# thedonutfactory/zig-tfhe

Hardware: AMD Instinct MI355X
Metric: gate-bootstraps/sec (NAND, 128-bit params) at 1/2/4/8 MI355X; % HBM roofline (higher is better)
Workload: dtype f64; 1 GPU; 1024 NAND gate bootstraps per GPU per step, SECURITY_128_BIT (n=700, N=1024, L=3, Bg=2^6, t=9); global_batch=1024, params=128, parallelism=dp1

## Files before the change

### zig-tfhe_amd/csrc/tfhe_kernels.hip

```cpp
#include <algorithm>
#include <string>
#include <type_traits>

#include "tfhe_device.hpp"

namespace tfhe {


constexpr int BO_GATES = 8;
constexpr int BO_LDS_BUF = 2048 * 4;
constexpr int BO_LDS_AT = 1024 * 2;
constexpr int BO_LDS_TOTAL = BR_LDS_BK + BR_LDS_TW + BR_LDS_TWIST + BO_GATES * (BO_LDS_BUF + BO_LDS_AT);
static_assert(BO_LDS_TOTAL <= 160 * 1024, "octo form LDS");
constexpr int BO_LDS_BUF_AT = BR_LDS_BK + BR_LDS_TW + BR_LDS_TWIST;
static_assert(BO_LDS_BUF_AT % 4096 == 0 && BO_LDS_BUF % 4096 == 0, "gather_rot needs 4 KB-aligned buffers");

DEV void issue_bk_pair_async512(const double2 *__restrict__ src, double2 *slot, int tid) {
    const uint32_t base = (uint32_t)(size_t)(lds_void_t *)slot + (uint32_t)(tid & ~63) * 16;
    const uint32_t voff = (uint32_t)tid * 16;
#pragma unroll
    for (int k = 0; k < 4; k++) {
        const uint32_t dst = __builtin_amdgcn_readfirstlane(base + 512 * 16 * k);
        const double2 *piece = src + 512 * k;
        uint32_t keep;
        asm volatile(
            "s_mov_b32 %0, m0\n\ts_mov_b32 m0, %2\n\ts_nop 0\n\tglobal_load_lds_dwordx4 %1, %3\n\ts_mov_b32 m0, %0"
            : "=&s"(keep)
            : "v"(voff), "s"(dst), "s"(piece)
            : "memory");
    }
}

template <bool FU>
DEV void load_digits_row_regs(C2 *d, const uint32_t *tA, const uint32_t *tB, int row, int L, int bgbit,
                              const C2 *twist_t) {
    const bool from_a = row < L;
    const int level = from_a ? row : row - L;
#pragma unroll
    for (int q = 0; q < 8; q++) {
        const int m = br3(q);
        const uint32_t x0 = from_a ? tA[m] : tB[m], x1 = from_a ? tA[m + 8] : tB[m + 8];
        d[q] = twist_in<FU>(digit_f64_flipped(x0, level, bgbit), digit_f64_flipped(x1, level, bgbit), twist_t[64 * m]);
    }
}

template <bool FU>
DEV void mac_row_lds(C2 *fa, C2 *fb, const C2 *d, const double2 *bk, int t) {
    double2 k[2][2];
    k[0][0] = bk[t];
    k[0][1] = bk[64 + t];
#pragma unroll
    for (int q = 0; q < 8; q++) {
        const int c = q & 1;
        if (q + 1 < 8) {
            k[c ^ 1][0] = bk[(2 * q + 2) * 64 + t];
            k[c ^ 1][1] = bk[(2 * q + 3) * 64 + t];
        }
        const C2 x = d[q];
        const double2 ka = k[c][0], kb = k[c][1];
        if (FU) {
            fa[q] = c2(fmad(x.x, ka.x, fmad(-x.y, ka.y, fa[q].x)), fmad(x.x, ka.y, fmad(x.y, ka.x, fa[q].y)));
            fb[q] = c2(fmad(x.x, kb.x, fmad(-x.y, kb.y, fb[q].x)), fmad(x.x, kb.y, fmad(x.y, kb.x, fb[q].y)));
        } else {
            const C2 ta = c2(x.x * ka.x - x.y * ka.y, x.x * ka.y + x.y * ka.x);
            const C2 tb = c2(x.x * kb.x - x.y * kb.y, x.x * kb.y + x.y * kb.x);
            fa[q] = c2(fa[q].x + ta.x, fa[q].y + ta.y);
            fb[q] = c2(fb[q].x + tb.x, fb[q].y + tb.y);
        }
    }
}

template <int L, bool FU>
DEV void octo_rows(const uint32_t *tA, const uint32_t *tB, int bgbit, const LdsTwAtPass &T, const C2 *twist_t,
                   C2 *xb, int t, int tid, C2 *fa, C2 *fb, double2 *s_bk, uint32_t k0,
                   const double2 *__restrict__ bkd, uint32_t pairs) {
#pragma unroll 1
    for (int r = 0; r < 2 * L; r++) {
        const uint32_t k = k0 + (uint32_t)(r >> 1);
        C2 d[1][8];
        load_digits_row_regs<FU>(d[0], tA, tB, r, L, bgbit, twist_t);
        fft512<1, false, FU, LdsTwAtPass, true>(d, xb, T, t);
        if ((r & 1) == 0) {
            asm volatile("s_waitcnt vmcnt(0)" ::: "memory");
            __syncthreads();
            if (k + 1 < pairs)
                issue_bk_pair_async512(bkd + (size_t)((k + 1) / L) * L * 2048 + (size_t)((k + 1) % L) * 2048,
                                       s_bk + ((k + 1) & 1) * 2048, tid);
        }
        mac_row_lds<FU>(fa, fb, d[0], s_bk + (k & 1) * 2048 + (r & 1) * 1024, t);
    }
}

template <int L, bool SMALL, bool FU, bool TV = false>
__global__ __launch_bounds__(512, 1) void k_blind_rotate_octo(
    KParams P, DevTables TT, const uint8_t *__restrict__ ops, const uint32_t *__restrict__ in_a,
    const uint32_t *__restrict__ in_b, const uint32_t *__restrict__ idx, const uint32_t *__restrict__ testvec,
    const double2 *__restrict__ bkd, uint32_t *__restrict__ out, int out_mode, size_t B) {
    __shared__ __attribute__((aligned(16))) unsigned char smem[BO_LDS_TOTAL];
    const int tid = threadIdx.x;
    const int t = tid & 63;
    const int w = __builtin_amdgcn_readfirstlane(tid >> 6);
    double2 *s_bk = reinterpret_cast<double2 *>(smem);
    C2 *s_tw = reinterpret_cast<C2 *>(smem + BR_LDS_BK);
    C2 *s_twist = reinterpret_cast<C2 *>(smem + BR_LDS_BK + BR_LDS_TW);
    unsigned char *gbase = smem + BR_LDS_BK + BR_LDS_TW + BR_LDS_TWIST;
    uint32_t *s_buf = reinterpret_cast<uint32_t *>(gbase + w * BO_LDS_BUF);
    C2 *s_x = reinterpret_cast<C2 *>(s_buf);
    uint16_t *s_at = reinterpret_cast<uint16_t *>(gbase + BO_GATES * BO_LDS_BUF + w * BO_LDS_AT);

    const int n = P.n;
    const size_t g_raw = (size_t)blockIdx.x * BO_GATES + w;
    const bool valid = g_raw < B;
    const size_t g = valid ? g_raw : B - 1;
    const size_t ia = idx ? idx[2 * g] : g, ib = idx ? idx[2 * g + 1] : g;
    const uint32_t *A = in_a + ia * (size_t)(n + 1);
    const uint32_t *Bv = in_b ? in_b + ib * (size_t)(n + 1) : A;
    const int op = ops ? (int)ops[g] : 255;
    const uint32_t pairs = (uint32_t)n * L;
    if constexpr (TV) testvec = item_testvec(P, testvec, g);

    if (lds_layout_bad(smem)) {
        if (tid == 0) __hip_atomic_fetch_or(P.err, (uint32_t)DEV_ERR_LDS_LAYOUT, __ATOMIC_RELAXED, __HIP_MEMORY_SCOPE_AGENT);
        return;
    }
    issue_bk_pair_async512(bkd, s_bk, tid);
    for (int x = tid; x < 511; x += 512) s_tw[x] = TT.tw[x];
    for (int x = tid; x < 512; x += 512) s_twist[x] = TT.twist[x];
    int bt = 0;
    for (int i = t; i <= n; i += 64) {
        const uint32_t c = gate_combine(op, A[i], Bv[i], i == n);
        const uint32_t tl = (uint32_t)(((uint64_t)c + (1ull << 20)) >> 21);
        if (i < n) s_at[i] = (uint16_t)tl;
        else bt = 2048 - (int)tl;
    }
    bt = __builtin_amdgcn_readlane(bt, n & 63);
    uint32_t accA[16], accB[16];
#pragma unroll
    for (int m = 0; m < 16; m++) {
        accA[m] = rot_read(testvec, t + 64 * m, bt);
        accB[m] = rot_read(testvec + 1024, t + 64 * m, bt);
        s_buf[t + 64 * m] = accA[m];
        s_buf[1024 + t + 64 * m] = accB[m];
    }
    __syncthreads();
    LdsTwAtPass T;
    T.init(s_tw, TT);
    const C2 *twist_t = s_twist + t;
    int at_next = s_at[0];
    uint32_t near = NEAR_NONE;
    const uint32_t msbs = digit_msbs(L, P.bgbit);
    const uint32_t buf_base = (uint32_t)(size_t)(lds_void_t *)s_buf;

    for (int i = 0; i < n; i++) {
        const int at = __builtin_amdgcn_readfirstlane(at_next);
        at_next = s_at[i + 1 < n ? i + 1 : i];
        uint32_t tA[16], tB[16];
        uint32_t xb[16];
        gather_rot(buf_base, t, at, xb, tA, tB);
        __builtin_amdgcn_sched_barrier(0);
#pragma unroll
        for (int m = 0; m < 16; m++) {
            const uint32_t sg = gather_sign(xb[m]), off_s = P.offset - sg;
            tA[m] = tmp_word(tA[m], sg, off_s, accA[m], msbs);
            tB[m] = tmp_word(tB[m], sg, off_s, accB[m], msbs);
        }
        wave_sync();
        C2 fa[8], fb[8];
#pragma unroll
        for (int q = 0; q < 8; q++) {
            fa[q] = c2(0.0, 0.0);
            fb[q] = c2(0.0, 0.0);
        }
        octo_rows<L, FU>(tA, tB, P.bgbit, T, twist_t, s_x, t, tid, fa, fb, s_bk, (uint32_t)(L * i), bkd, pairs);
        inverse_and_add<SMALL, 64, true, FU>(fa, fb, s_x, T, twist_t, t, accA, accB, near);
        wave_sync();
#pragma unroll
        for (int m = 0; m < 16; m++) {
            s_buf[t + 64 * m] = accA[m];
            s_buf[1024 + t + 64 * m] = accB[m];
        }
        wave_sync();
    }
    if (FU) near_tie_flag(P, near, g, valid);

    if (!valid) return;
    if (out_mode == BR_OUT_LV1) {
        uint32_t *o = out + g * (size_t)1025;
        for (int j = t; j <= 1024; j += 64) o[j] = j == 0 ? s_buf[0] : j < 1024 ? 0u - s_buf[1024 - j] : s_buf[1024];
    } else if (out_mode == BR_OUT_LV0_EXTRACT2) {
        uint32_t *o = out + g * (size_t)(n + 1);
        for (int j = t; j <= n; j += 64) o[j] = j == 0 ? s_buf[0] : j < n ? 0u - s_buf[n - j] : s_buf[1024];
    } else {
        uint32_t *o = out + g * (size_t)2048;
        for (int j = t; j < 2048; j += 64) o[j] = s_buf[j];
    }
}



constexpr size_t BR_WIDE_MAX_ITEMS = 512;
constexpr int WIDE_INV_W0 = 2;
constexpr int WIDE_ROW45_PRIO = 1;

template <int L, bool SMALL, bool FU = false, int RC = 0, bool TV = false>
__global__ __launch_bounds__(512, 1) void k_blind_rotate_wide(
    KParams P, DevTables TT, const uint8_t *__restrict__ ops, const uint32_t *__restrict__ in_a,
    const uint32_t *__restrict__ in_b, const uint32_t *__restrict__ idx, const uint32_t *__restrict__ testvec,
    const double2 *__restrict__ bkd, uint32_t *__restrict__ out, int out_mode, size_t B) {
    __shared__ __attribute__((aligned(16))) C2 s_tw[512];
    __shared__ __attribute__((aligned(16))) C2 s_twist[512];
    __shared__ __attribute__((aligned(16))) C2 s_prod[2][2 * L][512];
    __shared__ __attribute__((aligned(16))) uint32_t s_acc[2048];
    __shared__ uint16_t s_at[1024];
    __shared__ int s_bt;
    __shared__ uint32_t s_rows[8];
    static_assert(!RC || L == 3, "row counters: L = 3");
    const int tid = threadIdx.x;
    const int t = tid & 63;
    const int w = __builtin_amdgcn_readfirstlane(tid >> 6);
    const int n = P.n;
    const size_t g = blockIdx.x;
    const size_t ia = idx ? idx[2 * g] : g, ib = idx ? idx[2 * g + 1] : g;
    const uint32_t *A = in_a + ia * (size_t)(n + 1);
    const uint32_t *Bv = in_b ? in_b + ib * (size_t)(n + 1) : A;
    const int op = ops ? (int)ops[g] : 255;
    if constexpr (TV) testvec = item_testvec(P, testvec, g);
    const size_t trgsw = (size_t)2 * L * 1024;

    for (int x = tid; x < 511; x += 512) s_tw[x] = TT.tw[x];
    for (int x = tid; x < 512; x += 512) s_twist[x] = TT.twist[x];
    if (RC && tid < 8) s_rows[tid] = 0u;
    const int row = RC && w < 4 ? w ^ 2 : w;
    if (w == 0) {
        for (int i = t; i <= n; i += 64) {
            uint32_t c = gate_combine(op, A[i], Bv[i], i == n);
            uint32_t tl = (uint32_t)(((uint64_t)c + (1ull << 20)) >> 21);
            if (i < n) s_at[i] = (uint16_t)tl;
            else s_bt = 2048 - (int)tl;
        }
    }
    double2 kr[8][2];
    if (w < 2 * L) {
#pragma unroll
        for (int q = 0; q < 8; q++)
#pragma unroll
            for (int h = 0; h < 2; h++) kr[q][h] = bkd[((size_t)row * 8 + q) * 128 + h * 64 + t];
    }
    __syncthreads();
    const int bt = __builtin_amdgcn_readfirstlane(s_bt);
    if (w < 2) {
#pragma unroll
        for (int m = 0; m < 16; m++) s_acc[w * 1024 + t + 64 * m] = rot_read(testvec + w * 1024, t + 64 * m, bt);
    }
    LdsTw T;
    T.init(s_tw, TT);
    const C2 *twist_t = s_twist + t;
    __syncthreads();
    const int ipoly = w - WIDE_INV_W0;
    const bool is_inv = ipoly == 0 || ipoly == 1;
    const bool pf_late = !RC && w < 2 * L && !is_inv;
    uint32_t accr[16];
    if (is_inv) {
#pragma unroll
        for (int m = 0; m < 16; m++) accr[m] = s_acc[ipoly * 1024 + t + 64 * m];
    }

    if (RC ? (w == 0 || w == 1) : (w == 4 || w == 5)) __builtin_amdgcn_s_setprio(WIDE_ROW45_PRIO);
    uint32_t fail = 0;
    const uint32_t spin_cap = P.spin_cap ? P.spin_cap : BR_SPIN_CAP_DEFAULT;
    int at_next = s_at[0];
    uint32_t near = NEAR_NONE;
    PhaseProf pp;
    pp.start();
    for (int i = 0; i < n; i++) {
        pp.mark(0);
        const int at = __builtin_amdgcn_readfirstlane(at_next);
        at_next = s_at[i + 1 < n ? i + 1 : i];
        if (w < 2 * L) {
            const int poly = row >= L ? 1 : 0;
            const int level = row - poly * L;
            const uint32_t *pa = s_acc + poly * 1024;
            uint32_t rot[16], own[16];
            pp.mark(8);
            const int rb = (t - at) & 2047;
#pragma unroll
            for (int m = 0; m < 16; m++) {
                rot[m] = pa[(rb + 64 * m) & 1023];
                own[m] = pa[t + 64 * m];
            }
            __builtin_amdgcn_sched_barrier(0);
            pp.mark(9);
            C2 d[1][8];
            const uint32_t msbs = digit_msbs(L, P.bgbit);
#pragma unroll
            for (int q = 0; q < 8; q++) {
                const int m = br3(q);
                const bool n0 = ((rb + 64 * m) & 1024) != 0, n1 = ((rb + 64 * (m + 8)) & 1024) != 0;
                const uint32_t x0 = ((n0 ? 0u - rot[m] : rot[m]) - own[m] + P.offset) ^ msbs;
                const uint32_t x1 = ((n1 ? 0u - rot[m + 8] : rot[m + 8]) - own[m + 8] + P.offset) ^ msbs;
                d[0][q] = twist_in<FU>(digit_f64_flipped(x0, level, P.bgbit), digit_f64_flipped(x1, level, P.bgbit),
                                       twist_t[64 * m]);
            }
            pp.mark(10);
            fft512<1, false, FU>(d, s_prod[0][row], T, t);
            pp.mark(11);
#pragma unroll
            for (int q = 0; q < 8; q++) {
                s_prod[0][row][t + 64 * q] = cmul_bk<FU>(d[0][q], kr[q][0]);
                s_prod[1][row][t + 64 * q] = cmul_bk<FU>(d[0][q], kr[q][1]);
            }
            if (RC) {
                __builtin_amdgcn_sched_barrier(0);
                counter_add(s_rows + row);
            }
            pp.mark(14);
            if (i + 1 < n && !pf_late) wide_prefetch(kr, bkd + (size_t)(i + 1) * trgsw, row, t);
        }
        if (RC) {
            if (is_inv) {
                C2 fs[8];
                pp.mark(2);
#pragma unroll
                for (int r = 0; r < 2 * L; r++) {
                    uint32_t f = 0;
                    spin_until_ge<1>(s_rows + r, (uint32_t)i + 1u, spin_cap, f);
                    fail |= f;
                    __builtin_amdgcn_sched_barrier(0);
#pragma unroll
                    for (int q = 0; q < 8; q++) {
                        const C2 tq = s_prod[ipoly][r][t + 64 * q];
                        fs[q] = r == 0 ? tq : c2(fs[q].x + tq.x, fs[q].y + tq.y);
                    }
                }
                pp.mark(4);
                C2 e[1][8];
#pragma unroll
                for (int q = 0; q < 8; q++) e[0][q] = fs[br3(q)];
                C2 twr[8];
#pragma unroll
                for (int q = 0; q < 8; q++) twr[q] = twist_t[64 * q];
                pp.mark(12);
                fft512<1, true, FU>(e, s_prod[ipoly][0], T, t);
                pp.mark(13);
                uint32_t *pa = s_acc + ipoly * 1024;
#pragma unroll
                for (int q = 0; q < 8; q++) {
                    double re, im;
                    untwist_out<false, FU>(e[0][q], twr[q], re, im);
                    accr[q] += to_torus<SMALL, FU>(re, near);
                    accr[q + 8] += to_torus<SMALL, FU>(im, near);
                    pa[t + 64 * q] = accr[q];
                    pa[t + 64 * q + 512] = accr[q + 8];
                }
            }
            pp.mark(5);
            __syncthreads();
            continue;
        }
        pp.mark(1);
        __syncthreads();
        pp.mark(2);
        const int f = t + 64 * w;
        C2 fa = s_prod[0][0][f], fb = s_prod[1][0][f];
#pragma unroll
        for (int r = 1; r < 2 * L; r++) {
            const C2 ta = s_prod[0][r][f], tb = s_prod[1][r][f];
            fa = c2(fa.x + ta.x, fa.y + ta.y);
            fb = c2(fb.x + tb.x, fb.y + tb.y);
        }
        s_prod[0][0][f] = fa;
        s_prod[0][1][f] = fb;
        pp.mark(3);
        __syncthreads();
        pp.mark(4);
        if (pf_late && i + 1 < n) wide_prefetch(kr, bkd + (size_t)(i + 1) * trgsw, row, t);
        if (is_inv) {
            C2 e[1][8];
#pragma unroll
            for (int q = 0; q < 8; q++) e[0][q] = s_prod[0][ipoly][t + 64 * br3(q)];
            C2 twr[8];
#pragma unroll
            for (int q = 0; q < 8; q++) twr[q] = twist_t[64 * q];
            pp.mark(12);
            fft512<1, true, FU>(e, s_prod[0][ipoly], T, t);
            pp.mark(13);
            uint32_t *pa = s_acc + ipoly * 1024;
#pragma unroll
            for (int q = 0; q < 8; q++) {
                double re, im;
                untwist_out<false, FU>(e[0][q], twr[q], re, im);
                accr[q] += to_torus<SMALL, FU>(re, near);
                accr[q + 8] += to_torus<SMALL, FU>(im, near);
                pa[t + 64 * q] = accr[q];
                pa[t + 64 * q + 512] = accr[q + 8];
            }
        }
        pp.mark(5);
        __syncthreads();
    }
    pp.mark(6);
#ifdef TFHE_PHASE_PROF
    if (t == 0)
        pp.flush(g_phase_cycles + w * 16, 16);
#endif
    if (RC) report_wait_failure(P, fail, DEV_ERR_GATE_WAIT);
    if (FU) near_tie_flag(P, near, g, true);

    if (w != 0) return;
    if (out_mode == BR_OUT_LV1) {
        uint32_t *o = out + g * (size_t)1025;
        for (int j = t; j <= 1024; j += 64) o[j] = j == 0 ? s_acc[0] : j < 1024 ? 0u - s_acc[1024 - j] : s_acc[1024];
    } else if (out_mode == BR_OUT_LV0_EXTRACT2) {
        uint32_t *o = out + g * (size_t)(n + 1);
        for (int j = t; j <= n; j += 64) o[j] = j == 0 ? s_acc[0] : j < n ? 0u - s_acc[n - j] : s_acc[1024];
    } else {
        uint32_t *o = out + g * (size_t)2048;
        for (int j = t; j < 2048; j += 64) o[j] = s_acc[j];
    }
}


template <int T, int G>
__global__ __launch_bounds__(256) void k_key_switch_sel(KParams P, const uint32_t *__restrict__ lv1,
                                                        const uint32_t *__restrict__ ksk,
                                                        uint32_t *__restrict__ out, size_t B) {
    const size_t g0 = (size_t)blockIdx.y * G;
    const int w = blockIdx.x * 256 + threadIdx.x;
    const int lane = threadIdx.x & 63;
    const int n1 = P.n + 1;
    const bool active = w < n1;
    const int wc = active ? w : 0;
    uint32_t res[G];
#pragma unroll
    for (int g = 0; g < G; g++) res[g] = (w == P.n && g0 + g < B) ? lv1[(g0 + g) * 1025 + 1024] : 0u;
    const uint32_t prec = 1u << (32 - (1 + 2 * T));
    const size_t rs = (size_t)P.ks_stride;
    const size_t stride_i = (size_t)T * 4 * rs;
    const uint32_t *rows0 = ksk + wc;
    for (int i0 = 0; i0 < 1024; i0 += 64) {
        uint32_t pkv[G];
#pragma unroll
        for (int g = 0; g < G; g++) {
            const uint32_t a = (g0 + g < B) ? lv1[(g0 + g) * 1025 + i0 + lane] : 0u;
            pkv[g] = (a + prec) >> (32 - 2 * T);
        }
        for (int ii = 0; ii < 64; ii++) {
            const uint32_t *rows = rows0 + (size_t)(i0 + ii) * stride_i;
            uint32_t r[T][3];
#pragma unroll
            for (int j = 0; j < T; j++)
#pragma unroll
                for (int k = 0; k < 3; k++) r[j][k] = rows[(size_t)(4 * j + k + 1) * rs];
#pragma unroll
            for (int g = 0; g < G; g++) {
                const uint32_t pk = __builtin_amdgcn_readlane(pkv[g], ii);
#pragma unroll
                for (int j = 0; j < T; j++) {
                    const uint32_t k = (pk >> (2 * (T - 1 - j))) & 3u;
                    const uint32_t v = (k & 2u) ? ((k & 1u) ? r[j][2] : r[j][1]) : ((k & 1u) ? r[j][0] : 0u);
                    res[g] -= v;
                }
            }
        }
    }
    if (active) {
#pragma unroll
        for (int g = 0; g < G; g++)
            if (g0 + g < B) out[(g0 + g) * n1 + w] = res[g];
    }
}

template <int T, int G>
__global__ __launch_bounds__(256) void k_key_switch_gather(KParams P, const uint32_t *__restrict__ lv1,
                                                           const uint32_t *__restrict__ ksk,
                                                           uint32_t *__restrict__ out, size_t B) {
    const size_t g0 = (size_t)blockIdx.y * G;
    const int w = blockIdx.x * 256 + threadIdx.x;
    const int lane = threadIdx.x & 63;
    const int n1 = P.n + 1;
    const bool active = w < n1;
    const int wc = active ? w : 0;
    const int basebit = P.basebit, base = 1 << basebit;
    uint32_t res[G];
#pragma unroll
    for (int g = 0; g < G; g++) res[g] = (w == P.n && g0 + g < B) ? lv1[(g0 + g) * 1025 + 1024] : 0u;
    const uint32_t prec = 1u << (32 - (1 + basebit * T));
    const size_t rs = (size_t)P.ks_stride;
    const size_t stride_i = (size_t)T * base * rs;
    const uint32_t *rows0 = ksk + wc;
    for (int i0 = 0; i0 < 1024; i0 += 64) {
        uint32_t pkv[G];
#pragma unroll
        for (int g = 0; g < G; g++) {
            const uint32_t a = (g0 + g < B) ? lv1[(g0 + g) * 1025 + i0 + lane] : 0u;
            pkv[g] = (a + prec) >> (32 - basebit * T);
        }
#pragma unroll 2
        for (int ii = 0; ii < 64; ii++) {
            const uint32_t *rows = rows0 + (size_t)(i0 + ii) * stride_i;
            uint32_t v[G][T];
#pragma unroll
            for (int g = 0; g < G; g++) {
                const uint32_t pk = __builtin_amdgcn_readlane(pkv[g], ii);
#pragma unroll
                for (int j = 0; j < T; j++) {
                    const uint32_t k = (pk >> (basebit * (T - 1 - j))) & (uint32_t)(base - 1);
                    v[g][j] = rows[(size_t)(base * j + k) * rs];
                }
            }
#pragma unroll
            for (int g = 0; g < G; g++)
#pragma unroll
                for (int j = 0; j < T; j++) res[g] -= v[g][j];
        }
    }
    if (active) {
#pragma unroll
        for (int g = 0; g < G; g++)
            if (g0 + g < B) out[(g0 + g) * n1 + w] = res[g];
    }
}

constexpr int KG_WAVES = 8;
constexpr int KG_ITEMS = 64 * KG_WAVES;
typedef int kg_v4i __attribute__((ext_vector_type(4)));
typedef int kg_v16i __attribute__((ext_vector_type(16)));

__host__ __device__ __forceinline__ int kg_cb(int basebit) { return basebit == 2 ? 8 : 4; }
__host__ __device__ __forceinline__ int kg_ksteps(int basebit) { return basebit == 2 ? 1 : 4; }
__host__ __device__ __forceinline__ int kg_blocks(int n_in, int basebit) { return (n_in + kg_cb(basebit) - 1) / kg_cb(basebit); }
static size_t ks_gemm_bytes_w(int out_w, int n_in, int t, int basebit) {
    const size_t w32 = (size_t)(out_w + 31) / 32;
    return (size_t)t * kg_blocks(n_in, basebit) * w32 * kg_ksteps(basebit) * 4 * 1024;
}
size_t ks_gemm_bytes(const KParams &P, int n_in, int t, int basebit) { return ks_gemm_bytes_w(P.n + 1, n_in, t, basebit); }
__global__ void k_ksk_to_gemm(KParams P, const uint32_t *__restrict__ ksk, uint32_t *__restrict__ kg, size_t words,
                              int n_in, int t, int basebit, int out_w, int row_stride) {
    const size_t x = (size_t)blockIdx.x * blockDim.x + threadIdx.x;
    if (x >= words) return;
    const int w32 = (out_w + 31) / 32, nib = kg_blocks(n_in, basebit), ks = kg_ksteps(basebit);
    const int base = 1 << basebit;
    const int q = (int)(x & 3), lane = (int)((x >> 2) & 63), b = (int)((x >> 8) & 3);
    size_t r = x >> 10;
    const int st = (int)(r % ks);
    r /= ks;
    const int wt = (int)(r % w32);
    r /= w32;
    const int ib = (int)(r % nib), j = (int)(r / nib);
    const int h = lane >> 5, c = lane & 31, w = 32 * wt + c;
    const size_t rs = (size_t)row_stride;
    uint32_t v = 0;
#pragma unroll
    for (int e4 = 0; e4 < 4; e4++) {
        const int e = 4 * q + e4;
        const int i = basebit == 2 ? 8 * ib + 4 * h + (e >> 2) : 4 * ib + st;
        const int k = basebit == 2 ? (e & 3) : 16 * h + e;
        const uint32_t word =
            (w < out_w && i < n_in) ? ksk[((size_t)(base * t) * i + (size_t)base * j + k) * rs + w] : 0u;
        v |= (((word >> (8 * b)) & 255u) ^ 128u) << (8 * e4);
    }
    kg[x] = v;
}

template <int N>
DEV void kg_wait() {
    static_assert(N >= 0 && N <= 15, "kg_wait");
#define KG_W(n_) if constexpr (N == n_) asm volatile("s_waitcnt vmcnt(" #n_ ")" ::: "memory");
    KG_W(0) KG_W(1) KG_W(2) KG_W(3) KG_W(4) KG_W(5) KG_W(6) KG_W(7)
    KG_W(8) KG_W(9) KG_W(10) KG_W(11) KG_W(12) KG_W(13) KG_W(14) KG_W(15)
#undef KG_W
}

template <int T, int BASEBIT>
__global__ __launch_bounds__(64 * KG_WAVES, 1) void k_key_switch_gemm(KParams P, const uint32_t *__restrict__ lv1,
                                                                   const uint32_t *__restrict__ kg,
                                                                   uint32_t *__restrict__ part, size_t B,
                                                                   int ib_per_split, int n_in, int in_stride,
                                                                   int out_w) {
    constexpr int CB = BASEBIT == 2 ? 8 : 4;
    constexpr int KS = BASEBIT == 2 ? 1 : 4;
    constexpr int STEP_BYTES = KS * 4 * 1024;
    constexpr int WORDS_BYTES = CB * KG_ITEMS * 4;
    constexpr int WORD_DMAS = CB / 4;
    constexpr int BUF_BYTES = T * STEP_BYTES + WORDS_BYTES;
    constexpr int STAGES = 3 * BUF_BYTES <= 160 * 1024 ? 3 : 2;
    constexpr int LOADER_DMAS = T * KS + WORD_DMAS;
    constexpr int OTHER_DMAS = WORD_DMAS;
    static_assert(STAGES * BUF_BYTES <= 160 * 1024, "gemm key-switch LDS");
    __shared__ __attribute__((aligned(16))) unsigned char smem[STAGES * BUF_BYTES];
    const int tid = threadIdx.x, lane = tid & 63;
    const int v = __builtin_amdgcn_readfirstlane(tid >> 6);
    const bool loader = v < 4;
    const int w32 = (out_w + 31) / 32;
    const int wt = blockIdx.x;
    const int nib = kg_blocks(n_in, BASEBIT);
    const int ib_lo = blockIdx.z * ib_per_split, ib_hi = min(nib, ib_lo + ib_per_split);
    const size_t m_wg = (size_t)blockIdx.y * KG_ITEMS;
    const int h = lane >> 5, c = lane & 31;
    const uint32_t *a_src[WORD_DMAS];
#pragma unroll
    for (int r = 0; r < WORD_DMAS; r++) {
        const size_t m = m_wg + (CB == 8 ? 256 * r + (tid >> 1) : tid);
        a_src[r] = lv1 + (m < B ? m : B - 1) * (size_t)in_stride + (CB == 8 ? 4 * (tid & 1) : 0);
    }
    const uint32_t lds0 = (uint32_t)(size_t)(lds_void_t *)smem;
    auto issue = [&](int ib, int slot) {
        const uint32_t base = lds0 + slot * BUF_BYTES;
        if (loader) {
#pragma unroll
            for (int j = 0; j < T; j++)
#pragma unroll
                for (int st = 0; st < KS; st++) {
                    const uint32_t *src = kg + ((((size_t)j * nib + ib) * w32 + wt) * KS + st) * 1024 + tid * 4;
                    const uint32_t dst =
                        __builtin_amdgcn_readfirstlane(base + j * STEP_BYTES + st * 4096 + (tid & ~63) * 16);
                    uint32_t keep;
                    asm volatile(
                        "s_mov_b32 %0, m0\n\ts_mov_b32 m0, %2\n\ts_nop 0\n\tglobal_load_lds_dwordx4 %1, off\n\ts_mov_b32 m0, %0"
                        : "=&s"(keep)
                        : "v"(src), "s"(dst)
                        : "memory");
                }
        }
#pragma unroll
        for (int r = 0; r < WORD_DMAS; r++) {
            const uint32_t dst =
                __builtin_amdgcn_readfirstlane(base + T * STEP_BYTES + r * 256 * 32 + (tid & ~63) * 16);
            uint32_t keep;
            asm volatile(
                "s_mov_b32 %0, m0\n\ts_mov_b32 m0, %2\n\ts_nop 0\n\tglobal_load_lds_dwordx4 %1, off\n\ts_mov_b32 m0, %0"
                : "=&s"(keep)
                : "v"(a_src[r] + CB * ib), "s"(dst)
                : "memory");
        }
    };
    kg_v16i acc[2][4];
#pragma unroll
    for (int s = 0; s < 2; s++)
#pragma unroll
        for (int b = 0; b < 4; b++) acc[s][b] = kg_v16i{};
    const uint32_t prec = 1u << (32 - (1 + BASEBIT * T));
#pragma unroll
    for (int k = 0; k < STAGES - 1; k++)
        if (ib_lo + k < ib_hi) issue(ib_lo + k, k);
    for (int ib = ib_lo; ib < ib_hi; ib++) {
        const int slot = (ib - ib_lo) % STAGES;
        const int ahead = min(STAGES - 2, ib_hi - 1 - ib);
        if (ahead == 1) {
            if (loader) kg_wait<LOADER_DMAS>();
            else kg_wait<OTHER_DMAS>();
        } else {
            kg_wait<0>();
        }
        __syncthreads();
        if (ib + STAGES - 1 < ib_hi) issue(ib + STAGES - 1, (slot + STAGES - 1) % STAGES);
        const unsigned char *buf = smem + slot * BUF_BYTES;
        const uint32_t *words = reinterpret_cast<const uint32_t *>(buf + T * STEP_BYTES);
        if constexpr (BASEBIT == 2) {
            uint32_t pk[2][4];
#pragma unroll
            for (int s = 0; s < 2; s++) {
                const kg_v4i wv = *reinterpret_cast<const kg_v4i *>(words + (64 * v + 32 * s + c) * 8 + 4 * h);
#pragma unroll
                for (int q = 0; q < 4; q++) pk[s][q] = ((uint32_t)wv[q] + prec) >> (32 - 2 * T);
            }
#pragma unroll
            for (int j = 0; j < T; j++) {
                kg_v4i a[2];
#pragma unroll
                for (int s = 0; s < 2; s++)
#pragma unroll
                    for (int q = 0; q < 4; q++)
                        a[s][q] = (int)(1u << (8u * ((pk[s][q] >> (2 * (T - 1 - j))) & 3u)));
#pragma unroll
                for (int b = 0; b < 4; b++) {
                    const kg_v4i bf = *reinterpret_cast<const kg_v4i *>(buf + j * STEP_BYTES + b * 1024 + lane * 16);
#pragma unroll
                    for (int s = 0; s < 2; s++)
                        acc[s][b] = __builtin_amdgcn_mfma_i32_32x32x32_i8(a[s], bf, acc[s][b], 0, 0, 0);
                }
            }
        } else {
            uint32_t pk[2][4];
#pragma unroll
            for (int s = 0; s < 2; s++) {
                const kg_v4i wv = *reinterpret_cast<const kg_v4i *>(words + (64 * v + 32 * s + c) * 4);
#pragma unroll
                for (int q = 0; q < 4; q++) pk[s][q] = ((uint32_t)wv[q] + prec) >> (32 - BASEBIT * T);
            }
#pragma unroll
            for (int j = 0; j < T; j++)
#pragma unroll
                for (int st = 0; st < KS; st++) {
                    kg_v4i a[2];
#pragma unroll
                    for (int s = 0; s < 2; s++) {
                        const uint32_t d = (pk[s][st] >> (BASEBIT * (T - 1 - j))) & 31u;
                        const uint32_t one = 1u << (8u * (d & 3u));
                        const int word = (int)(d >> 2) - 4 * h;
#pragma unroll
                        for (int q = 0; q < 4; q++) a[s][q] = word == q ? (int)one : 0;
                    }
#pragma unroll
                    for (int b = 0; b < 4; b++) {
                        const kg_v4i bf = *reinterpret_cast<const kg_v4i *>(buf + j * STEP_BYTES + st * 4096 +
                                                                            b * 1024 + lane * 16);
#pragma unroll
                        for (int s = 0; s < 2; s++)
                            acc[s][b] = __builtin_amdgcn_mfma_i32_32x32x32_i8(a[s], bf, acc[s][b], 0, 0, 0);
                    }
                }
        }
    }
    const int n1 = out_w;
    uint32_t *pz = part + (size_t)blockIdx.z * B * n1;
    const int w = 32 * wt + c;
    const size_t m_base = m_wg + 64 * v;
#pragma unroll
    for (int s = 0; s < 2; s++)
#pragma unroll
        for (int reg = 0; reg < 16; reg++) {
            const size_t m = m_base + 32 * s + (reg & 3) + 8 * (reg >> 2) + 4 * h;
            const uint32_t val = (uint32_t)acc[s][0][reg] + ((uint32_t)acc[s][1][reg] << 8) +
                                 ((uint32_t)acc[s][2][reg] << 16) + ((uint32_t)acc[s][3][reg] << 24);
            if (m < B && w < n1) pz[m * n1 + w] = val;
        }
}

__global__ void k_ks_gemm_reduce(KParams P, const uint32_t *__restrict__ lv1, const uint32_t *__restrict__ part,
                                 uint32_t *__restrict__ out, size_t B, int splits, int n_in, int in_stride, int t,
                                 int basebit) {
    const int n1 = P.n + 1;
    const size_t x = (size_t)blockIdx.x * blockDim.x + threadIdx.x;
    if (x >= B * n1) return;
    const size_t m = x / n1;
    const int w = (int)(x % n1);
    uint32_t r = (uint32_t)(kg_cb(basebit) * kg_blocks(n_in, basebit) * t) * 128u * 0x01010101u;
    for (int z = 0; z < splits; z++) r += part[(size_t)z * B * n1 + x];
    out[x] = (w == P.n ? lv1[m * (size_t)in_stride + n_in] : 0u) - r;
}

__global__ void k_ksk_zero_k0(uint32_t *__restrict__ ksk, int rs, int base, size_t groups) {
    size_t idx = (size_t)blockIdx.x * blockDim.x + threadIdx.x;
    if (idx >= groups * rs) return;
    size_t grp = idx / rs, x = idx % rs;
    ksk[grp * base * rs + x] = 0u;
}

constexpr int KL_CHUNK = 32;
constexpr int KL_WAVES = 4;
constexpr int KL_CHUNK_WIDE = 44;
constexpr int KL_WAVES_WIDE = 8;

template <int T, int BASEBIT, int CHUNK = KL_CHUNK, int WAVES = KL_WAVES, int GW = 1>
__global__ __launch_bounds__(64 * WAVES) void k_key_switch_lanes(KParams P, const uint32_t *__restrict__ lv1,
                                                          const uint32_t *__restrict__ ksk,
                                                          uint32_t *__restrict__ out, size_t B, int n_in,
                                                          int in_stride) {
    constexpr int BASE = 1 << BASEBIT;
    constexpr int PIECES = CHUNK / 4;
    constexpr int SLOTS = T * PIECES * BASE;
    constexpr int NDMA = (SLOTS + 63) / 64;
    constexpr int BUF = NDMA * 64 + 16;
    constexpr int RING = 2 * BUF;
    constexpr int RED = WAVES * CHUNK * 64;
    constexpr int LDS_BYTES = (RING * 16 * WAVES > RED * 4) ? RING * 16 * WAVES : RED * 4;
    static_assert(LDS_BYTES <= 160 * 1024, "key-switch LDS");
    __shared__ __attribute__((aligned(16))) unsigned char smem[LDS_BYTES];
    const int lane = threadIdx.x & 63;
    const int w = __builtin_amdgcn_readfirstlane(threadIdx.x >> 6);
    constexpr int IW = WAVES / GW;
    static_assert(WAVES % GW == 0, "GW divides WAVES");
    const int gw = w % GW, iw = w / GW;
    uint4 *ring = reinterpret_cast<uint4 *>(smem) + w * RING;
    const size_t g_raw = (size_t)blockIdx.y * (64 * GW) + gw * 64 + lane;
    const bool valid = g_raw < B;
    const size_t g = valid ? g_raw : B - 1;
    const int w0 = blockIdx.x * CHUNK;
    const size_t rs = (size_t)P.ks_stride;
    const size_t step_i = (size_t)BASE * T * rs;
    const int per = (n_in + IW - 1) / IW;
    const int ilo = min(n_in, iw * per), ihi = min(n_in, ilo + per);
    uint32_t src_off[NDMA];
#pragma unroll
    for (int c = 0; c < NDMA; c++) {
        const int sl = min(c * 64 + lane, SLOTS - 1);
        const int k = sl % BASE, piece = (sl / BASE) % PIECES, j = sl / (BASE * PIECES);
        src_off[c] = (uint32_t)((BASE * j + k) * rs + w0 + 4 * piece);
    }
    const uint32_t ring_lds = (uint32_t)(size_t)(lds_void_t *)ring;
    const uint32_t *a_src = lv1 + g * (size_t)in_stride;
    auto issue = [&](int i, int which) {
        const uint32_t *r = ksk + (size_t)i * step_i;
#pragma unroll
        for (int c = 0; c < NDMA; c++) {
            const uint32_t dst = __builtin_amdgcn_readfirstlane(ring_lds + (which * BUF + c * 64) * 16);
            uint32_t keep;
            asm volatile(
                "s_mov_b32 %0, m0\n\ts_mov_b32 m0, %2\n\ts_nop 0\n\tglobal_load_lds_dwordx4 %1, off\n\ts_mov_b32 m0, %0"
                : "=&s"(keep)
                : "v"(r + src_off[c]), "s"(dst)
                : "memory");
        }
        const uint32_t dst = __builtin_amdgcn_readfirstlane(ring_lds + (which * BUF + NDMA * 64) * 16);
        uint32_t keep;
        asm volatile(
            "s_mov_b32 %0, m0\n\ts_mov_b32 m0, %2\n\ts_nop 0\n\tglobal_load_lds_dword %1, off\n\ts_mov_b32 m0, %0"
            : "=&s"(keep)
            : "v"(a_src + i), "s"(dst)
            : "memory");
    };
    const uint32_t prec = 1u << (32 - (1 + BASEBIT * T));
    uint32_t acc[CHUNK];
#pragma unroll
    for (int x = 0; x < CHUNK; x++) acc[x] = 0u;
    if (ilo < ihi) issue(ilo, 0);
    for (int i = ilo; i < ihi; i++) {
        const int cur = (i - ilo) & 1;
        asm volatile("s_waitcnt vmcnt(0)" ::: "memory");
        wave_sync();
        if (i + 1 < ihi) issue(i + 1, cur ^ 1);
        const uint4 *buf = ring + cur * BUF;
        const uint32_t a = reinterpret_cast<const uint32_t *>(buf + NDMA * 64)[lane];
        const uint32_t pk = (a + prec) >> (32 - BASEBIT * T);
#pragma unroll
        for (int j = 0; j < T; j++) {
            const uint32_t k = (pk >> (BASEBIT * (T - 1 - j))) & (uint32_t)(BASE - 1);
            const uint4 *sl = buf + j * PIECES * BASE + k;
#pragma unroll
            for (int pc = 0; pc < PIECES; pc++) {
                const uint4 v = sl[pc * BASE];
                acc[4 * pc + 0] -= v.x;
                acc[4 * pc + 1] -= v.y;
                acc[4 * pc + 2] -= v.z;
                acc[4 * pc + 3] -= v.w;
            }
        }
        asm volatile("s_waitcnt lgkmcnt(0)" ::: "memory");
    }
    __syncthreads();
    uint32_t *red = reinterpret_cast<uint32_t *>(smem);
#pragma unroll
    for (int x = 0; x < CHUNK; x++) red[(w * CHUNK + x) * 64 + lane] = acc[x];
    __syncthreads();
    const int n1 = P.n + 1;
    for (int x = iw; x < CHUNK; x += IW) {
        uint32_t r = 0u;
#pragma unroll
        for (int v = 0; v < IW; v++) r += red[((v * GW + gw) * CHUNK + x) * 64 + lane];
        const int word = w0 + x;
        if (valid && word < n1) out[g * n1 + word] = (word == P.n ? a_src[n_in] : 0u) + r;
    }
}

constexpr int KS_RING_DEPTH = 4;
template <int N>
DEV void wait_vmcnt_le() {
    static_assert(N >= 0 && N < 64, "vmcnt field");
    __builtin_amdgcn_s_waitcnt((N & 15) | (7 << 4) | (15 << 8) | ((N >> 4) << 14));
}
template <int T, int BASEBIT, int CHUNK, int GW, int DEPTH>
__global__ __launch_bounds__(64 * GW) void k_key_switch_ring(KParams P, const uint32_t *__restrict__ lv1,
                                                           const uint32_t *__restrict__ ksk,
                                                           uint32_t *__restrict__ out, size_t B, int n_in,
                                                           int in_stride) {
    constexpr int BASE = 1 << BASEBIT;
    constexpr int PIECES = CHUNK / 4;
    constexpr int SLOTS = T * PIECES * BASE;
    static_assert(SLOTS % 64 == 0, "whole DMA instructions");
    constexpr int NDMA = SLOTS / 64;
    constexpr int MINE = (NDMA + GW - 1) / GW;
    constexpr int BUF = SLOTS + GW * 16;
    static_assert(DEPTH >= 3 && (MINE + 1) * (DEPTH - 2) < 64, "ring depth");
    __shared__ __attribute__((aligned(16))) uint4 ring[DEPTH * BUF];
    const int lane = threadIdx.x & 63;
    const int gw = __builtin_amdgcn_readfirstlane(threadIdx.x >> 6);
    const size_t g_raw = (size_t)blockIdx.y * (64 * GW) + gw * 64 + lane;
    const bool valid = g_raw < B;
    const size_t g = valid ? g_raw : B - 1;
    const int w0 = blockIdx.x * CHUNK;
    const size_t rs = (size_t)P.ks_stride;
    const size_t step_i = (size_t)BASE * T * rs;
    uint32_t src_off[MINE];
#pragma unroll
    for (int cc = 0; cc < MINE; cc++) {
        const int sl = ((cc * GW + gw) % NDMA) * 64 + lane;
        const int k = sl % BASE, piece = (sl / BASE) % PIECES, j = sl / (BASE * PIECES);
        src_off[cc] = (uint32_t)((BASE * j + k) * rs + w0 + 4 * piece);
    }
    const uint32_t ring_lds = (uint32_t)(size_t)(lds_void_t *)ring;
    const uint32_t *a_src = lv1 + g * (size_t)in_stride;
    auto issue = [&](int i, int slot) {
        const uint32_t *r = ksk + (size_t)i * step_i;
#pragma unroll
        for (int cc = 0; cc < MINE; cc++) {
            const uint32_t dst = __builtin_amdgcn_readfirstlane(ring_lds + (slot * BUF + ((cc * GW + gw) % NDMA) * 64) * 16);
            uint32_t keep;
            asm volatile(
                "s_mov_b32 %0, m0\n\ts_mov_b32 m0, %2\n\ts_nop 0\n\tglobal_load_lds_dwordx4 %1, off\n\ts_mov_b32 m0, %0"
                : "=&s"(keep)
                : "v"(r + src_off[cc]), "s"(dst)
                : "memory");
        }
        const uint32_t dst = __builtin_amdgcn_readfirstlane(ring_lds + (slot * BUF + SLOTS + gw * 16) * 16);
        uint32_t keep;
        asm volatile(
            "s_mov_b32 %0, m0\n\ts_mov_b32 m0, %2\n\ts_nop 0\n\tglobal_load_lds_dword %1, off\n\ts_mov_b32 m0, %0"
            : "=&s"(keep)
            : "v"(a_src + i), "s"(dst)
            : "memory");
    };
    const uint32_t prec = 1u << (32 - (1 + BASEBIT * T));
    uint32_t acc[CHUNK];
#pragma unroll
    for (int x = 0; x < CHUNK; x++) acc[x] = 0u;
    for (int i = 0; i < DEPTH - 1 && i < n_in; i++) issue(i, i);
    for (int i = 0; i < n_in; i++) {
        if (i + DEPTH - 2 < n_in) wait_vmcnt_le<(MINE + 1) * (DEPTH - 2)>();
        else wait_vmcnt_le<0>();
        asm volatile("s_waitcnt lgkmcnt(0)\n\ts_barrier" ::: "memory");
        if (i + DEPTH - 1 < n_in) issue(i + DEPTH - 1, (i + DEPTH - 1) % DEPTH);
        const uint4 *buf = ring + (i % DEPTH) * BUF;
        const uint32_t a = reinterpret_cast<const uint32_t *>(buf + SLOTS + gw * 16)[lane];
        const uint32_t pk = (a + prec) >> (32 - BASEBIT * T);
#pragma unroll
        for (int j = 0; j < T; j++) {
            const uint32_t k = (pk >> (BASEBIT * (T - 1 - j))) & (uint32_t)(BASE - 1);
            const uint4 *sl = buf + j * PIECES * BASE + k;
#pragma unroll
            for (int pc = 0; pc < PIECES; pc++) {
                const uint4 v = sl[pc * BASE];
                acc[4 * pc + 0] -= v.x;
                acc[4 * pc + 1] -= v.y;
                acc[4 * pc + 2] -= v.z;
                acc[4 * pc + 3] -= v.w;
            }
        }
    }
    const int n1 = P.n + 1;
    if (!valid) return;
#pragma unroll
    for (int x = 0; x < CHUNK; x++) {
        const int word = w0 + x;
        if (word < n1) out[g * n1 + word] = (word == P.n ? a_src[n_in] : 0u) + acc[x];
    }
}

__global__ __launch_bounds__(64) void k_fft_forward(DevTables TT, const uint32_t *__restrict__ in,
                                                    double *__restrict__ out) {
    __shared__ C2 s_x[512];
    const int t = threadIdx.x;
    const uint32_t *x = in + (size_t)blockIdx.x * 1024;
    RegTw T;
    T.init(TT.tw, t);
    C2 d[1][8];
#pragma unroll
    for (int q = 0; q < 8; q++) {
        int k = t + 64 * br3(q);
        d[0][q] = twist_in((double)(int32_t)x[k], (double)(int32_t)x[k + 512], TT.twist[k]);
    }
    fft512<1, false>(d, s_x, T, t);
    double *o = out + (size_t)blockIdx.x * 1024;
#pragma unroll
    for (int q = 0; q < 8; q++) {
        o[t + 64 * q] = d[0][q].x * 2.0;
        o[512 + t + 64 * q] = d[0][q].y * 2.0;
    }
}

__global__ __launch_bounds__(64) void k_fft_inverse(DevTables TT, const double *__restrict__ in,
                                                    uint32_t *__restrict__ out) {
    __shared__ C2 s_x[512];
    const int t = threadIdx.x;
    const double *f = in + (size_t)blockIdx.x * 1024;
    RegTw T;
    T.init(TT.tw, t);
    C2 d[1][8];
#pragma unroll
    for (int q = 0; q < 8; q++) {
        int k = t + 64 * br3(q);
        d[0][q] = c2(f[k], f[k + 512]);
    }
    fft512<1, true>(d, s_x, T, t);
    uint32_t *o = out + (size_t)blockIdx.x * 1024;
#pragma unroll
    for (int q = 0; q < 8; q++) {
        double tr, ti;
        untwist_out(d[0][q], TT.twist[t + 64 * q], tr, ti);
        o[t + 64 * q] = torus_from_f64(tr);
        o[512 + t + 64 * q] = torus_from_f64(ti);
    }
}

__global__ __launch_bounds__(64) void k_poly_mul(DevTables TT, const uint32_t *__restrict__ a,
                                                 const uint32_t *__restrict__ b, size_t b_stride,
                                                 uint32_t *__restrict__ out) {
    __shared__ C2 s_x[2 * 512];
    const int t = threadIdx.x;
    const uint32_t *x = a + (size_t)blockIdx.x * 1024;
    const uint32_t *y = b + (size_t)blockIdx.x * b_stride;
    RegTw T;
    T.init(TT.tw, t);
    C2 twl[8];
#pragma unroll
    for (int m = 0; m < 8; m++) twl[m] = TT.twist[t + 64 * m];
    C2 d[2][8];
#pragma unroll
    for (int q = 0; q < 8; q++) {
        int m = br3(q), k = t + 64 * m;
        d[0][q] = twist_in((double)(int32_t)x[k], (double)(int32_t)x[k + 512], twl[m]);
        d[1][q] = twist_in((double)(int32_t)y[k], (double)(int32_t)y[k + 512], twl[m]);
    }
// ... 639 lines not shown
```

Baseline: 175,000 gate-bootstraps/s.

## Use sparse SMFMAC int8 instructions for one-hot keyswitch GEMM

Replaces the dense 32x32x32 int8 MFMA in the keyswitch GEMM with the structured-sparse 32x32x64 SMFMAC. Because the A operand holds one-hot digit encodings, two digit steps (base-2^2) or two k-steps (base-2^5) can be packed into one sparse instruction with index metadata, roughly halving the matrix instruction count. In exchange it adds bit manipulation to build the compressed A values and sparsity indices, plus wider B fragment loads from LDS. Correctness depends on the intricate index encoding matching the hardware's 4:2 sparsity layout.

```diff
diff --git a/zig-tfhe_amd/csrc/ks_sparse.hpp b/zig-tfhe_amd/csrc/ks_sparse.hpp
--- /dev/null
+++ b/zig-tfhe_amd/csrc/ks_sparse.hpp
@@ -0,0 +1,58 @@
+#pragma once
+#include <cstdint>
+
+#if defined(__HIPCC__) || defined(__CUDACC__)
+#define KS_SPARSE_HD __host__ __device__ inline __attribute__((always_inline))
+#else
+#define KS_SPARSE_HD inline
+#endif
+
+struct KsSparseA {
+    uint32_t a[4];
+    uint32_t idx;
+};
+
+template <int T>
+KS_SPARSE_HD KsSparseA ks_sparse_a_bb2(const uint32_t (&pk)[4], int j0, bool two) {
+    constexpr uint32_t EVEN = (1u << (2 * T)) / 3;
+    uint32_t m[4], kc[4];
+    for (int g = 0; g < 4; g++) {
+        m[g] = pk[g] & (pk[g] >> 1) & EVEN;
+        kc[g] = pk[g] ^ (m[g] * 3u);
+    }
+    const uint32_t mm[2] = {(m[0] & 0xffffu) | (m[1] << 16), (m[2] & 0xffffu) | (m[3] << 16)};
+    auto pair = [&](int half, int sh) {
+        const uint32_t u = sh < 16 ? (mm[half] >> sh) & 0x10001u
+                                   : ((m[2 * half] >> sh) & 1u) | (((m[2 * half + 1] >> sh) & 1u) << 16);
+        return 0x00010001u + 0xffu * u;
+    };
+    KsSparseA r;
+    const int sh = 2 * (T - 1 - j0) - (two ? 2 : 0);
+    uint32_t y = 0;
+    for (int g = 0; g < 4; g++) y |= ((kc[g] >> sh) & (two ? 0xfu : 0x3u)) << (4 * g);
+    r.a[0] = pair(0, sh);
+    r.a[1] = pair(1, sh);
+    if (two) {
+        r.idx = ((y | y << 14) & 0x33333333u) | 0xccccccccu;
+        r.a[2] = pair(0, sh + 2);
+        r.a[3] = pair(1, sh + 2);
+    } else {
+        r.idx = y | 0xccccccccu;
+        r.a[2] = r.a[3] = 0;
+    }
+    return r;
+}
+
+KS_SPARSE_HD KsSparseA ks_sparse_a_bb5(uint32_t d0, uint32_t d1, int h) {
+    KsSparseA r;
+    r.idx = 0xccccccccu;
+    const uint32_t d[2] = {d0, d1};
+    for (int st = 0; st < 2; st++) {
+        const uint32_t k = d[st] & 3u, g = (d[st] >> 2) - 4u * (uint32_t)h;
+        const uint32_t hw = k == 3u ? 0x0100u : 0x0001u;
+        r.a[2 * st] = g < 2u ? hw << (16 * g) : 0u;
+        r.a[2 * st + 1] = (g & ~1u) == 2u ? hw << (16 * (g - 2u)) : 0u;
+        if (g < 4u && k != 3u) r.idx |= k << (16 * st + 4 * g);
+    }
+    return r;
+}
diff --git a/zig-tfhe_amd/csrc/tfhe_kernels.hip b/zig-tfhe_amd/csrc/tfhe_kernels.hip
--- a/zig-tfhe_amd/csrc/tfhe_kernels.hip
+++ b/zig-tfhe_amd/csrc/tfhe_kernels.hip
@@ -2,6 +2,7 @@
 #include <string>
 #include <type_traits>
 
+#include "ks_sparse.hpp"
 #include "tfhe_device.hpp"
 
 namespace tfhe {
@@ -524,6 +525,7 @@
 constexpr int KG_WAVES = 8;
 constexpr int KG_ITEMS = 64 * KG_WAVES;
 typedef int kg_v4i __attribute__((ext_vector_type(4)));
+typedef int kg_v8i __attribute__((ext_vector_type(8)));
 typedef int kg_v16i __attribute__((ext_vector_type(16)));
 
 __host__ __device__ __forceinline__ int kg_cb(int basebit) { return basebit == 2 ? 8 : 4; }
@@ -656,6 +658,10 @@
         if (ib + STAGES - 1 < ib_hi) issue(ib + STAGES - 1, (slot + STAGES - 1) % STAGES);
         const unsigned char *buf = smem + slot * BUF_BYTES;
         const uint32_t *words = reinterpret_cast<const uint32_t *>(buf + T * STEP_BYTES);
+        auto bfrag = [&](const unsigned char *bp) {
+            const kg_v4i lo = *reinterpret_cast<const kg_v4i *>(bp), hi = *reinterpret_cast<const kg_v4i *>(bp + 512);
+            return kg_v8i{lo[0], lo[1], lo[2], lo[3], hi[0], hi[1], hi[2], hi[3]};
+        };
         if constexpr (BASEBIT == 2) {
             uint32_t pk[2][4];
 #pragma unroll
@@ -665,19 +671,20 @@
                 for (int q = 0; q < 4; q++) pk[s][q] = ((uint32_t)wv[q] + prec) >> (32 - 2 * T);
             }
 #pragma unroll
-            for (int j = 0; j < T; j++) {
-                kg_v4i a[2];
-#pragma unroll
-                for (int s = 0; s < 2; s++)
-#pragma unroll
-                    for (int q = 0; q < 4; q++)
-                        a[s][q] = (int)(1u << (8u * ((pk[s][q] >> (2 * (T - 1 - j))) & 3u)));
+            for (int j0 = 0; j0 < T; j0 += 2) {
+                const bool two = j0 + 1 < T;
+                KsSparseA a[2];
+#pragma unroll
+                for (int s = 0; s < 2; s++) a[s] = ks_sparse_a_bb2<T>(pk[s], j0, two);
+                const unsigned char *bp = buf + (two ? j0 + 1 - h : j0) * STEP_BYTES + c * 16;
 #pragma unroll
                 for (int b = 0; b < 4; b++) {
-                    const kg_v4i bf = *reinterpret_cast<const kg_v4i *>(buf + j * STEP_BYTES + b * 1024 + lane * 16);
+                    const kg_v8i bf = bfrag(bp + b * 1024);
 #pragma unroll
                     for (int s = 0; s < 2; s++)
-                        acc[s][b] = __builtin_amdgcn_mfma_i32_32x32x32_i8(a[s], bf, acc[s][b], 0, 0, 0);
+                        acc[s][b] = __builtin_amdgcn_smfmac_i32_32x32x64_i8(
+                            kg_v4i{(int)a[s].a[0], (int)a[s].a[1], (int)a[s].a[2], (int)a[s].a[3]}, bf, acc[s][b],
+                            (int)a[s].idx, 0, 0);
                 }
             }
         } else {
@@ -691,23 +698,21 @@
 #pragma unroll
             for (int j = 0; j < T; j++)
 #pragma unroll
-                for (int st = 0; st < KS; st++) {
-                    kg_v4i a[2];
-#pragma unroll
-                    for (int s = 0; s < 2; s++) {
-                        const uint32_t d = (pk[s][st] >> (BASEBIT * (T - 1 - j))) & 31u;
-                        const uint32_t one = 1u << (8u * (d & 3u));
-                        const int word = (int)(d >> 2) - 4 * h;
-#pragma unroll
-                        for (int q = 0; q < 4; q++) a[s][q] = word == q ? (int)one : 0;
-                    }
+                for (int st = 0; st < KS; st += 2) {
+                    KsSparseA a[2];
+#pragma unroll
+                    for (int s = 0; s < 2; s++)
+                        a[s] = ks_sparse_a_bb5((pk[s][st] >> (BASEBIT * (T - 1 - j))) & 31u,
+                                               (pk[s][st + 1] >> (BASEBIT * (T - 1 - j))) & 31u, h);
+                    const unsigned char *bp = buf + j * STEP_BYTES + (st + h) * 4096 + c * 16;
 #pragma unroll
                     for (int b = 0; b < 4; b++) {
-                        const kg_v4i bf = *reinterpret_cast<const kg_v4i *>(buf + j * STEP_BYTES + st * 4096 +
-                                                                            b * 1024 + lane * 16);
+                        const kg_v8i bf = bfrag(bp + b * 1024);
 #pragma unroll
                         for (int s = 0; s < 2; s++)
-                            acc[s][b] = __builtin_amdgcn_mfma_i32_32x32x32_i8(a[s], bf, acc[s][b], 0, 0, 0);
+                            acc[s][b] = __builtin_amdgcn_smfmac_i32_32x32x64_i8(
+                                kg_v4i{(int)a[s].a[0], (int)a[s].a[1], (int)a[s].a[2], (int)a[s].a[3]}, bf,
+                                acc[s][b], (int)a[s].idx, 0, 0);
                     }
                 }
         }
```

Result: no change. 174,900 gate-bootstraps/s, median of 2 (-0.0%).
